# infil00p/openbts-ttsou

Measured on AMD Instinct MI355X. Metric: Mbursts/s (156.25-sym @ 4 sps) demod+detect, higher is better.
Workload: dtype f32

## Files before the change

openbts-ttsou_amd/csrc/trxsig_corr.h:

```cpp
#pragma once
#include "trxsig_dev.h"

namespace {

template <int SPS>
struct CorrGeom {
  static constexpr int NL = 36 * SPS;
  static constexpr int NC = (NL + 15) / 16;
  static constexpr int FRONT = 8 * SPS;
  static constexpr int WPAD0 = NC * 16 + 15 * SPS + 1;
  static constexpr int WPAD = ((WPAD0 + 15) / 32) * 32 + 16;
  static constexpr int H = (5 * SPS + 1 > 12) ? 5 * SPS + 1 : 12;
  static constexpr int NS = 2 * H + 1;
  static constexpr int NE = 20 * SPS;
  static constexpr int NEQ = (NE + 15) / 16;
  static constexpr int NPAIR = (NS + 2) / 2;
};
template <typename T>
__device__ __forceinline__ T &rec_slot(T *rec, int Bpad, int s, int b) { return rec[2 * ((size_t)(s >> 1) * Bpad + b) + (s & 1)]; }

template <int N>
__device__ __forceinline__ float add_row_shl(float acc, float v) {
  float r;
  if (N == 0) asm volatile("v_add_f32 %0, %1, %2" : "=v"(r) : "v"(v), "v"(acc));
  else asm volatile("v_add_f32_dpp %0, %1, %2 row_shl:%3 row_mask:0xf bank_mask:0xf bound_ctrl:1"
                    : "=v"(r) : "v"(v), "v"(acc), "n"(N));
  return r;
}
template <int SPS, int I>
__device__ __forceinline__ float energy_chain_step(float acc, const float (&nrm)[CorrGeom<SPS>::NEQ]) {
  if constexpr (I < CorrGeom<SPS>::NE) {
    acc = add_row_shl<I % 16>(acc, nrm[I / 16]);
    return energy_chain_step<SPS, I + 1>(acc, nrm);
  } else {
    return acc;
  }
}
template <int SPS, int I>
__device__ __forceinline__ float energy_chain(float acc, const float (&nrm)[CorrGeom<SPS>::NEQ]) {
  asm volatile("s_nop 1");
  return energy_chain_step<SPS, I>(acc, nrm);
}

template <int SPS>
struct CorrIn {
  typedef CorrGeom<SPS> G;
  static constexpr int NW = (CorrGeom<SPS>::NL + 15) / 16;
  cx w[NW];
  cx e[CorrGeom<SPS>::NEQ];
  int b;
  bool live, good;
  __device__ __forceinline__ void stage_window(cx *W, int r) const {
#pragma unroll
    for (int i = 0; i < NW; i++) {
      const int q = r + 16 * i;
      if (q < G::NL) W[G::FRONT + q] = w[i];
    }
  }
  __device__ __forceinline__ void stage_norms(float *ef, int r) const {
#pragma unroll
    for (int q = 0; q < G::NEQ; q++) {
      const int i = r + 16 * q;
      if (i < G::NE) ef[i] = norm2(e[q]);
    }
  }
};

template <int SPS>
__device__ __forceinline__ void corr_issue(CorrIn<SPS> &in, int b, int B, int r, const cx *__restrict__ samples,
                                           const int32_t *__restrict__ offset, const int32_t *__restrict__ length) {
  typedef CorrGeom<SPS> G;
  in.b = b;
  in.live = b < B;
  int off = 0, len = 0;
  if (in.live) { off = offset[b]; len = length[b]; }
  in.good = in.live && (off >= 0) && (len >= 92 * SPS) && (len <= 157 * SPS) && (len % SPS == 0);
  const cx *x = samples + (in.good ? off : 0);
#pragma unroll
  for (int i = 0; i < CorrIn<SPS>::NW; i++) {
    const int q = r + 16 * i;
    in.w[i] = (in.good && q < G::NL) ? x[56 * SPS + q] : mk(0, 0);
  }
#pragma unroll
  for (int q = 0; q < G::NEQ; q++) {
    const int i = r + 16 * q;
    in.e[q] = (in.good && i < G::NE) ? x[i] : mk(0, 0);
  }
}

template <int SPS, bool REC, bool EFIRST = false, unsigned TAPCLS = TRX_TAPS_GENERIC, typename IN = CorrIn<SPS>>
__device__ __forceinline__ void corr_round(const IN &in, cx *W, float4 *E, int lane, int r, const cx (&tap)[16],
                                           cx *__restrict__ rec, int Bpad, int &M_out, float &energy_out) {
  typedef CorrGeom<SPS> G;
  auto stage_norms = [&] { in.stage_norms(reinterpret_cast<float *>(E), r); };
  auto sum_norms = [&] {
    float energy = 0.0f;
#pragma unroll
    for (int i4 = 0; i4 < (G::NE + 3) / 4; i4++) {
      const float4 e = E[i4];
      energy = energy + e.x;
      if (4 * i4 + 1 < G::NE) energy = energy + e.y;
      if (4 * i4 + 2 < G::NE) energy = energy + e.z;
      if (4 * i4 + 3 < G::NE) energy = energy + e.w;
    }
    return energy;
  };
  float energy = 0.0f;
  if (EFIRST) {
    stage_norms();
    wave_lds_fence();
    energy = sum_norms();
    asm volatile("" : "+v"(energy));
    wave_lds_fence();
  }
  for (int q = r; q < G::FRONT; q += 16) W[q] = mk(0, 0);
  for (int q = G::FRONT + G::NL + r; q < G::WPAD; q += 16) W[q] = mk(0, 0);
  in.stage_window(W, r);
  if (!EFIRST) stage_norms();
  wave_lds_fence();
  if (!EFIRST) energy = sum_norms();

  float bestP = 0.0f;
  int bestT = -1;
  cx cval[G::NC];
  constexpr int CG = (SPS == 4) ? TRX_CORR_CG : 1;
  constexpr int UPC = 16 / SPS;
  constexpr int NU = UPC * (CG - 1) + 16;
#pragma unroll
  for (int c0 = 0; c0 < G::NC; c0 += CG) {
    cx sv[NU];
#pragma unroll
    for (int u = 0; u < NU; u++) sv[u] = W[r + 16 * c0 + SPS * u];
#pragma unroll
    for (int cc = 0; cc < CG; cc++) {
      if (c0 + cc < G::NC) {
        cx acc = mk(0, 0);
#pragma unroll
        for (int k = 15; k >= 0; k--) acc = cadd(acc, cmul_tap(sv[UPC * cc + k], tap[k], (TAPCLS >> (2 * k)) & 3));
        cval[c0 + cc] = acc;
      }
    }
  }
  wave_lds_fence();
#pragma unroll
  for (int c = 0; c < G::NC; c++) {
    const int t = r + 16 * c;
    if (t < G::NL) {
      W[t] = cval[c];
      const float p = norm2(cval[c]);
      if (p > bestP) { bestP = p; bestT = t; }
    }
  }
#pragma unroll
  for (int m = 1; m < 16; m <<= 1) {
    const float oP = __shfl_xor(bestP, m, 64);
    const int oT = __shfl_xor(bestT, m, 64);
    const bool take = (oP > bestP) || (oP == bestP && oT >= 0 && (bestT < 0 || oT < bestT));
    if (take) { bestP = oP; bestT = oT; }
  }
  wave_lds_fence();

  M_out = bestT;
  energy_out = energy;
  if (REC && in.live) {
    const int M = bestT;
    auto slot = [&](int s) {
      cx v = mk(0, 0);
      if (s < G::NS) {
        const int lag = M - G::H + s;
        if (lag >= 0 && lag < G::NL) v = W[lag];
      } else if (s == G::NS) {
        v = mk(__int_as_float(in.good ? M : -2), energy);
      }
      return v;
    };
    for (int j = r; j < G::NPAIR; j += 16) {
      const cx a = slot(2 * j), c = slot(2 * j + 1);
      reinterpret_cast<float4 *>(rec)[(size_t)j * Bpad + in.b] = make_float4(a.r, a.i, c.r, c.i);
    }
  }
  wave_lds_fence();
  (void)lane;
}


inline unsigned tap_classes(const TrxTables *hT, int tsc) {
  unsigned m = 0;
  for (int k = 0; k < 16; k++) {
    const trx_c32 a = hT->mid_ctap[tsc][k];
    const unsigned c = (a.r == 1.0f || a.r == -1.0f) ? 1u : ((a.i == 1.0f || a.i == -1.0f) ? 2u : 0u);
    m |= c << (2 * k);
  }
  return m;
}

}
```

openbts-ttsou_amd/csrc/trxsig_dev.h:

```cpp
#pragma once
#include <hip/hip_runtime.h>
#include <hip/hip_fp16.h>
#include <stdint.h>

#include <type_traits>

#include "trxsig_tables.h"
#include "trxsig_launch.h"

#ifndef TRX_CORR_CG
#define TRX_CORR_CG 3
#endif
#ifndef TRX_CORR_WPS
#define TRX_CORR_WPS 1
#endif
#ifndef TRX_CORR_ROUNDS
#define TRX_CORR_ROUNDS 1
#endif
#ifndef TRX_DEMOD_WAVES
#define TRX_DEMOD_WAVES 4
#endif

namespace {

typedef trx_c32 cx;

__device__ __forceinline__ cx mk(float r, float i) { cx z; z.r = r; z.i = i; return z; }
__device__ __forceinline__ cx cmul(cx x, cx a) { return mk(x.r * a.r - x.i * a.i, x.r * a.i + x.i * a.r); }
__device__ __forceinline__ cx cmulr(cx x, float a) { return mk(x.r * a, x.i * a); }
__device__ __forceinline__ cx cadd(cx x, cx a) { return mk(x.r + a.r, x.i + a.i); }
__device__ __forceinline__ float norm2(cx x) { return x.i * x.i + x.r * x.r; }
__device__ __forceinline__ cx cinv(cx x) { float n = norm2(x); return mk(x.r / n, -x.i / n); }
__device__ __forceinline__ cx cdiv(cx x, cx a) { return cmul(x, cinv(a)); }

template <int CTRL>
__device__ __forceinline__ float dpp_f(float v) {
  return __int_as_float(__builtin_amdgcn_update_dpp(0, __float_as_int(v), CTRL, 0xf, 0xf, true));
}
template <int CTRL>
__device__ __forceinline__ int dpp_i(int v) { return __builtin_amdgcn_update_dpp(0, v, CTRL, 0xf, 0xf, true); }
__device__ __forceinline__ float wave_sum_any_order(float v) {
  v += dpp_f<0xB1>(v);
  v += dpp_f<0x4E>(v);
  v += dpp_f<0x141>(v);
  v += dpp_f<0x140>(v);
  const float r0 = __int_as_float(__builtin_amdgcn_readlane(__float_as_int(v), 0));
  const float r1 = __int_as_float(__builtin_amdgcn_readlane(__float_as_int(v), 16));
  const float r2 = __int_as_float(__builtin_amdgcn_readlane(__float_as_int(v), 32));
  const float r3 = __int_as_float(__builtin_amdgcn_readlane(__float_as_int(v), 48));
  return ((r0 + r1) + r2) + r3;
}
__device__ __forceinline__ void argmax_take(float &P, int &T, float oP, int oT) {
  const bool take = (oP > P) || (oP == P && oT >= 0 && (T < 0 || oT < T));
  P = take ? oP : P;
  T = take ? oT : T;
}
__device__ __forceinline__ void wave_argmax(float &P, int &T) {
  argmax_take(P, T, dpp_f<0xB1>(P), dpp_i<0xB1>(T));
  argmax_take(P, T, dpp_f<0x4E>(P), dpp_i<0x4E>(T));
  argmax_take(P, T, dpp_f<0x141>(P), dpp_i<0x141>(T));
  argmax_take(P, T, dpp_f<0x140>(P), dpp_i<0x140>(T));
  float bp = __int_as_float(__builtin_amdgcn_readlane(__float_as_int(P), 0));
  int bt = __builtin_amdgcn_readlane(T, 0);
#pragma unroll
  for (int r = 16; r < 64; r += 16)
    argmax_take(bp, bt, __int_as_float(__builtin_amdgcn_readlane(__float_as_int(P), r)), __builtin_amdgcn_readlane(T, r));
  P = bp; T = bt;
}

typedef float v2f __attribute__((ext_vector_type(2)));
__device__ __forceinline__ v2f pk(cx z) { v2f v = {z.r, z.i}; return v; }
__device__ __forceinline__ v2f pk_cmul(v2f x, v2f a) {
  v2f p, q, r;
  asm("v_pk_mul_f32 %0, %1, %2 op_sel_hi:[0,1]" : "=v"(p) : "v"(x), "v"(a));
  asm("v_pk_mul_f32 %0, %1, %2 op_sel:[1,1] op_sel_hi:[1,0]" : "=v"(q) : "v"(x), "v"(a));
  asm("v_pk_add_f32 %0, %1, %2 neg_lo:[0,1]" : "=v"(r) : "v"(p), "v"(q));
  return r;
}
__device__ __forceinline__ v2f pk_mul(v2f x, v2f a) {
  v2f r;
  asm("v_pk_mul_f32 %0, %1, %2" : "=v"(r) : "v"(x), "v"(a));
  return r;
}
template <int HI>
__device__ __forceinline__ v2f pk_mul_tap(v2f x, v2f t) {
  v2f r;
  if (HI) asm("v_pk_mul_f32 %0, %1, %2 op_sel:[0,1] op_sel_hi:[1,1]" : "=v"(r) : "v"(x), "v"(t));
  else asm("v_pk_mul_f32 %0, %1, %2 op_sel_hi:[1,0]" : "=v"(r) : "v"(x), "v"(t));
  return r;
}
__device__ __forceinline__ v2f pk_csub(v2f x, v2f a) {
  v2f r;
  asm("v_pk_add_f32 %0, %1, %2 neg_lo:[0,1] neg_hi:[0,1]" : "=v"(r) : "v"(x), "v"(a));
  return r;
}
__device__ __forceinline__ cx unpk(v2f v) { return mk(v.x, v.y); }
__device__ __forceinline__ v2f pk_cadd(v2f x, v2f a) {
  v2f r;
  asm("v_pk_add_f32 %0, %1, %2" : "=v"(r) : "v"(x), "v"(a));
  return r;
}

struct SmpC32 {
  static constexpr int kBytes = 8;
  static __device__ __forceinline__ cx ld(const void *base, long long i) { return reinterpret_cast<const cx *>(base)[i]; }
  typedef cx raw_t;
  static __device__ __forceinline__ raw_t ldraw(const void *base, long long i) { return reinterpret_cast<const cx *>(base)[i]; }
  static __device__ __forceinline__ raw_t zero() { return mk(0, 0); }
  static __device__ __forceinline__ cx widen(raw_t r) { return r; }
  static __device__ __forceinline__ float4 ld2(const void *base, long long first, int q) {
    return reinterpret_cast<const float4 *>(reinterpret_cast<const cx *>(base) + first)[q];
  }
};
struct SmpF16 {
  static constexpr int kBytes = 4;
  static __device__ __forceinline__ cx ld(const void *base, long long i) {
    const float2 v = __half22float2(reinterpret_cast<const __half2 *>(base)[i]);
    return mk(v.x, v.y);
  }
  typedef unsigned raw_t;
  static __device__ __forceinline__ raw_t ldraw(const void *base, long long i) { return reinterpret_cast<const unsigned *>(base)[i]; }
  static __device__ __forceinline__ raw_t zero() { return 0u; }
  static __device__ __forceinline__ cx widen(raw_t r) {
    const float2 v = __half22float2(*reinterpret_cast<const __half2 *>(&r));
    return mk(v.x, v.y);
  }
  static __device__ __forceinline__ float4 ld2(const void *base, long long first, int q) {
    const uint2 u = reinterpret_cast<const uint2 *>(reinterpret_cast<const __half2 *>(base) + first)[q];
    const float2 a = __half22float2(*reinterpret_cast<const __half2 *>(&u.x)), b = __half22float2(*reinterpret_cast<const __half2 *>(&u.y));
    return make_float4(a.x, a.y, b.x, b.y);
  }
};

struct TapArg { float v[32]; };

#define TRX_TAPS_GENERIC 0u
template <int SPS> struct TapPattern {
  static constexpr unsigned value = (SPS == 4) ? 0x19999999u : 0x99999999u;
};
__device__ __forceinline__ float fma_steer(float a, float b, float c) {
  float r;
  asm("v_fma_f32 %0, %1, %2, %3 ; steering" : "=v"(r) : "v"(a), "v"(b), "v"(c));
  return r;
}
__device__ __forceinline__ float fma_steer_s(float a, float b_sgpr, float c) {
  float r;
  asm("v_fma_f32 %0, %1, %2, %3 ; steering" : "=v"(r) : "v"(a), "s"(b_sgpr), "v"(c));
  return r;
}
__device__ __forceinline__ cx cmul_tap(cx x, cx a, int cls) {
  if (cls == 1) {
    const float p = x.i * a.i, q = x.r * a.i;
    cx z;
    asm("v_fma_f32 %0, %2, %4, -%5 ; exact-product\n\tv_fma_f32 %1, %3, %4, %6 ; exact-product"
        : "=&v"(z.r), "=v"(z.i) : "v"(x.r), "v"(x.i), "s"(a.r), "v"(p), "v"(q));
    return z;
  }
  if (cls == 2) {
    const float p = x.r * a.r, q = x.i * a.r;
    cx z;
    asm("v_fma_f32 %0, %3, -%4, %5 ; exact-product\n\tv_fma_f32 %1, %2, %4, %6 ; exact-product"
        : "=&v"(z.r), "=v"(z.i) : "v"(x.r), "v"(x.i), "s"(a.i), "v"(p), "v"(q));
    return z;
  }
  return cmul(x, a);
}

#define TRX_PI_F 3.14159274101257324f
#define TRX_2PI_F 6.28318548202514648f

template <int N>
__device__ __forceinline__ float row_shl(float v) {
  if (N == 0) return v;
  return __int_as_float(__builtin_amdgcn_update_dpp(0, __float_as_int(v), 0x100 + N, 0xf, 0xf, true));
}

__device__ __forceinline__ void lds_barrier() {
  asm volatile("s_waitcnt lgkmcnt(0)\n\ts_barrier" ::: "memory");
}
__device__ __forceinline__ void wave_lds_fence() {
  __builtin_amdgcn_fence(__ATOMIC_RELEASE, "wavefront");
  __builtin_amdgcn_wave_barrier();
  __builtin_amdgcn_fence(__ATOMIC_ACQUIRE, "wavefront");
}

__device__ __forceinline__ float dev_range_reduce(float arg) {
  if (arg > 1.0F) arg = arg - (ceilf(arg) - 1.0F);
  if (arg < 0.0F) arg = arg + ceilf(-arg);
  return arg;
}
__device__ __forceinline__ float dev_sin_lookup(const float *__restrict__ sinT, float x) {
  const float arg = dev_range_reduce(x * (1 / TRX_2PI_F));
  const float argT = arg * (float)TRX_TABLESIZE;
  int argI = (int)argT;
  argI = argI < 0 ? 0 : (argI > TRX_TABLESIZE ? TRX_TABLESIZE : argI);
  const float delta = argT - argI;
  const float iDelta = 1.0F - delta;
  return iDelta * sinT[argI] + delta * sinT[argI + 1];
}
#define TRX_FSHIFT_MAXPHASE 25000.0f
__device__ __forceinline__ cx dev_expj_lookup(const TrxTables *__restrict__ T, float x) {
  const float arg = dev_range_reduce(x * (1 / TRX_2PI_F));
  const float argT = arg * (float)TRX_TABLESIZE;
  int argI = (int)argT;
  argI = argI < 0 ? 0 : (argI > TRX_TABLESIZE ? TRX_TABLESIZE : argI);
  const float delta = argT - argI;
  const float iDelta = 1.0F - delta;
  return mk(iDelta * T->cosT[argI] + delta * T->cosT[argI + 1], iDelta * T->sinT[argI] + delta * T->sinT[argI + 1]);
}
__device__ __forceinline__ float dev_sinc(const float *__restrict__ sinT, float x) {
  if ((x >= 0.01F) || (x <= -0.01F)) return dev_sin_lookup(sinT, x) / x;
  return 1.0F;
}

}
```

openbts-ttsou_amd/csrc/trxsig_normal.hip:

```cpp
#include "trxsig_bisect.h"
#include "trxsig_corr.h"
#include "trxsig_demod.h"
#include "trxsig_rxgen.h"

#ifndef TRX_RXC_WPS
#define TRX_RXC_WPS 1
#endif
#ifndef TRX_RXD_WPS
#define TRX_RXD_WPS 1
#endif

namespace {

template <int SPS, unsigned TAPCLS>
__global__ __launch_bounds__(256, TRX_CORR_WPS) void k_tsc_corr(const TrxTables *__restrict__ T,
                                                  const cx *__restrict__ samples,
                                                  const int32_t *__restrict__ offset,
                                                  const int32_t *__restrict__ length, int B, TapArg taps,
                                                  cx *__restrict__ rec, int Bpad) {
  typedef CorrGeom<SPS> G;
  static_assert(8 * G::WPAD >= 4 * G::NE, "the energy norms are staged in the row itself");
  __shared__ __attribute__((aligned(16))) cx rows[16][G::WPAD];
  (void)T;
  const int lane = threadIdx.x & 63, wave = threadIdx.x >> 6;
  const int row = lane >> 4, r = lane & 15;
  const int slot = wave * 4 + row;

  cx tap[16];
#pragma unroll
  for (int k = 0; k < 16; k++) tap[k] = mk(taps.v[2 * k], taps.v[2 * k + 1]);

  typedef CorrIn<SPS> In;
  In in[TRX_CORR_ROUNDS];
#pragma unroll
  for (int i = 0; i < TRX_CORR_ROUNDS; i++)
    corr_issue<SPS>(in[i], (blockIdx.x * TRX_CORR_ROUNDS + i) * 16 + slot, B, r, samples, offset, length);
#pragma unroll
  for (int i = 0; i < TRX_CORR_ROUNDS; i++) {
    int M;
    float energy;
    corr_round<SPS, true, true, TAPCLS, In>(in[i], rows[slot], reinterpret_cast<float4 *>(rows[slot]), lane, r, tap, rec, Bpad, M, energy);
  }
}


#ifdef TRX_TUNING_BUILD
template <int SPS>
__global__ __launch_bounds__(64) void k_tsc_peak(const TrxTables *__restrict__ T,
                                                 const cx *__restrict__ rec, int Bpad, int B, int tsc,
                                                 float detect_thresh, float energy_thresh,
                                                 uint8_t *__restrict__ flags, cx *__restrict__ amp_out,
                                                 float *__restrict__ toa_out,
                                                 float *__restrict__ avgpwr_out) {
  typedef CorrGeom<SPS> G;
  __shared__ cx loc[26][64];
  __shared__ float pw[G::NS][64];
  const int lane = threadIdx.x;
  const int b = blockIdx.x * 64 + lane;
  const bool live = b < B;
  const int bb = live ? b : B - 1;

  const cx meta = rec_slot(rec, Bpad, G::NS, bb);
  const int M = __float_as_int(meta.r);
  const float energy = meta.i;
  const bool good = M != -2;
#pragma unroll
  for (int s = 0; s < G::NS; s++) {
    const cx v = rec_slot(rec, Bpad, s, bb);
    pw[s][lane] = norm2(v);
    const int j = s - (G::H - 12);
    if (j >= 0 && j < 24) {
      const int lag = M - 12 + j;
      loc[j][lane] = (lag > G::NL - 2) ? mk(0, 0) : v;
    }
  }
  loc[24][lane] = mk(0, 0);
  loc[25][lane] = mk(0, 0);

  float peakIx;
  const cx peak = peak_bisect<64>(T->sinc_grid, loc, lane, M, &peakIx);

  float toa = peakIx;
  cx amp = peak;
  bool detected = false;
  const bool energy_ok = good && (energy_thresh < 0.0f ||
                                  energy / (float)(unsigned)G::NE > energy_thresh * energy_thresh);
  if (!(toa < 0.0f) && !(toa > (float)G::NL) && good) {
    const int p = (int)rintf(toa);
    float valley = 0.0f;
    int numRms = 0;
#pragma unroll
    for (int i = 2 * SPS; i <= 5 * SPS; i++) {
      const int lo = p - i, hi = p + i;
      int slo = lo - M + G::H, shi = hi - M + G::H;
      slo = slo < 0 ? 0 : slo; shi = shi > G::NS - 1 ? G::NS - 1 : shi;
      const float vlo = pw[slo][lane], vhi = pw[shi][lane];
      if (lo >= 0) { valley += vlo; numRms++; }
      if (hi < G::NL) { valley += vhi; numRms++; }
    }
    if (numRms < 2) {
      amp = mk(0, 0);
    } else {
      const float RMS = (float)((double)sqrtf(valley / (float)numRms) + 0.00001);
      const float peakToMean = sqrtf(norm2(amp)) / RMS;
      amp = cdiv(amp, T->mid_gain[tsc]);
      toa = toa - T->mid_toa[tsc];
      toa = toa - (float)((66 - 56) * SPS);
      detected = peakToMean > detect_thresh;
    }
  } else {
    amp = mk(0, 0);
  }
  if (!energy_ok) { amp = mk(0, 0); toa = 0.0f; detected = false; }

  if (live) {
    uint8_t fl = 0;
    if (!good) fl = TRXSIG_F_BADLEN;
    else fl = (energy_ok ? TRXSIG_F_ENERGY : 0) | (detected ? TRXSIG_F_DETECT : 0);
    flags[b] = fl;
    amp_out[b] = amp;
    toa_out[b] = toa;
    if (avgpwr_out) avgpwr_out[b] = good ? energy / (float)(unsigned)G::NE : 0.0f;
  }
}


template <int SPS>
struct Peak8Geom {
  typedef CorrGeom<SPS> G;
  static constexpr int NV = 2 * (3 * SPS + 1);
  static constexpr int O_PW = 26 * 2;
  static constexpr int O_V = O_PW + ((G::NS + 3) & ~3);
  static constexpr int STRIDE = O_V + ((NV + 3) & ~3);
};

template <int SPS>
__global__ __launch_bounds__(256, 8) void k_tsc_peak8(const TrxTables *__restrict__ T, const cx *__restrict__ rec, int Bpad,
                                                   int B, cx gain_inv, float mid_toa, float detect_thresh,
                                                   float energy_thresh, uint8_t *__restrict__ flags,
                                                   cx *__restrict__ amp_out, float *__restrict__ toa_out,
                                                   float *__restrict__ avgpwr_out) {
  typedef CorrGeom<SPS> G;
  typedef Peak8Geom<SPS> P8;
  __shared__ __attribute__((aligned(16))) float stab[32][24];
  __shared__ __attribute__((aligned(16))) float scratch[32][P8::STRIDE];
  {
    float tv[3];
#pragma unroll
    for (int k = 0; k < 3; k++) { const int ix = threadIdx.x * 3 + k; tv[k] = T->sinc_grid[16 * (ix / 24)][ix % 24]; }
#pragma unroll
    for (int k = 0; k < 3; k++) { const int ix = threadIdx.x * 3 + k; stab[ix / 24][ix % 24] = tv[k]; }
  }
  const int lane = threadIdx.x & 63;
  const int r = lane & 7;
  const int slot = threadIdx.x >> 3;
  const int b = blockIdx.x * 32 + slot;
  const bool live = b < B;
  const int bb = live ? b : B - 1;
  float *S = scratch[slot];
  cx *loc = reinterpret_cast<cx *>(S);
  float *pw = S + P8::O_PW, *V = S + P8::O_V;

  const cx meta = rec_slot(rec, Bpad, G::NS, bb);
  const int M = __float_as_int(meta.r);
  const float energy = meta.i;
  const bool good = M != -2;
#pragma unroll
  for (int s0 = 0; s0 < G::NS; s0 += 8) {
    const int sl = s0 + r;
    if (sl < G::NS) {
      const cx v = rec_slot(rec, Bpad, sl, bb);
      pw[sl] = norm2(v);
      const int j = sl - (G::H - 12);
      if (j >= 0 && j < 24) loc[j] = (M - 12 + j > G::NL - 2) ? mk(0, 0) : v;
    }
  }
  if (r < 2) loc[24 + r] = mk(0, 0);
  __syncthreads();

  int e = 0;
  asm volatile("" : "+v"(e));
  bool active = true;
  cx peak = mk(0, 0);
  {
    const int rel2 = kFusedRel2.v[r], rel1 = kFusedRel1.v[r];
#pragma unroll
    for (int st = 0; st < 4; st++) {
      const int inc_last = 128 >> (2 * st);
      const int el = e + (rel2 >> 2) * inc_last;
      float srow[24];
      if (st < 3) {
        const float4 *rw = reinterpret_cast<const float4 *>(stab[(el & 511) >> 4]);
#pragma unroll
        for (int q = 0; q < 6; q++) {
          const float4 t4 = rw[q];
          srow[4 * q] = t4.x; srow[4 * q + 1] = t4.y; srow[4 * q + 2] = t4.z; srow[4 * q + 3] = t4.w;
        }
      } else {
        fused_row(T, el, srow);
      }
      const cx pt = fused_point(loc, el, rel2 & 3, srow);
      fused_decide<8, 2, false>(pt, lane, 2 * inc_last, e, active, peak);
    }
    {
      float srow[24];
      fused_row(T, e, srow);
      const cx pt = fused_point(loc, e, rel1 & 3, srow);
      fused_decide<8, 1, false>(pt, lane, 1, e, active, peak);
    }
    float srow[24];
    fused_row(T, e, srow);
    peak = fused_point(loc, e, 1, srow);
    asm volatile("" : "+v"(peak.r), "+v"(peak.i));
  }
  cx amp;
  float toa;
  bool detected, energy_ok;
  fused_tail<SPS, 8>([&](int lag) { const int sl = lag - M + G::H; return (sl < 0 || sl >= G::NS) ? 0.0f : pw[sl]; }, V, r, M, e,
                     peak, good, energy, gain_inv, mid_toa, detect_thresh, energy_thresh, amp, toa, detected, energy_ok);
  if (live && r == 0) {
    uint8_t fl = 0;
    if (!good) fl = TRXSIG_F_BADLEN;
    else fl = (energy_ok ? TRXSIG_F_ENERGY : 0) | (detected ? TRXSIG_F_DETECT : 0);
    flags[b] = fl;
    amp_out[b] = amp;
    toa_out[b] = toa;
    if (avgpwr_out) avgpwr_out[b] = good ? energy / (float)(unsigned)G::NE : 0.0f;
  }
}



#endif

#ifndef TRX_PEAK2_THREADS
#define TRX_PEAK2_THREADS 512
#endif
constexpr int kPeak2Threads = TRX_PEAK2_THREADS;
template <int SPS>
__global__ __launch_bounds__(kPeak2Threads) void k_tsc_peak2(const TrxTables *__restrict__ T, const cx *__restrict__ rec, int Bpad,
                                                   int B, cx gain_inv, float mid_toa, float detect_thresh,
                                                   float energy_thresh, uint8_t *__restrict__ flags,
                                                   cx *__restrict__ amp_out, float *__restrict__ toa_out,
                                                   float *__restrict__ avgpwr_out) {
  typedef CorrGeom<SPS> G;
  constexpr int NL = G::NL, NE = G::NE, NP = 3 * SPS + 3;
  __shared__ __attribute__((aligned(16))) SincLds stab;
  const int tid = threadIdx.x;
  const int h = tid & 1;
  const int b = blockIdx.x * (kPeak2Threads / 2) + (tid >> 1);
  const bool live = b < B;
  const int bb = live ? b : B - 1;
#ifdef TRX_PEAK_PROBE
  long long pt_[16] = {0};
  int pk_ = 0;
#define TRX_STAMP() pt_[pk_++] = clock64()
#else
#define TRX_STAMP()
#endif
  TRX_STAMP();

  float4 tv[3072 / kPeak2Threads];
  sinc_lds_issue<kPeak2Threads>(T, tid, tv);
  const cx meta = rec_slot(rec, Bpad, G::NS, bb);
  const int M = __float_as_int(meta.r);
  const float energy = meta.i;
  const bool good = M != -2;
  const float4 *rec4 = reinterpret_cast<const float4 *>(rec);
  cx q[23];
  {
    constexpr int S0 = G::H - 12, P0 = S0 >> 1;
    float4 pw[12];
#pragma unroll
    for (int i = 0; i < 12; i++) pw[i] = rec4[(size_t)(P0 + h + i) * Bpad + bb];
#pragma unroll
    for (int k = 0; k < 23; k++) {
      const int ix = k + 2 * h;
      const float4 p4 = pw[((S0 + k) >> 1) - P0];
      const cx v = ((S0 + k) & 1) ? mk(p4.z, p4.w) : mk(p4.x, p4.y);
      q[k] = (M - 12 + ix > NL - 2) ? mk(0, 0) : v;
    }
  }
  cx vmine_[NP];
  constexpr int VLO = G::H - (5 * SPS + 1), VHI = G::H + (2 * SPS - 1);
  if constexpr ((VLO & 1) == 0 && (VHI & 1) == 0) {
    float4 pv[(NP + 1) / 2];
#pragma unroll
    for (int i = 0; i < (NP + 1) / 2; i++) pv[i] = rec4[(size_t)(((h ? VHI : VLO) >> 1) + i) * Bpad + bb];
#pragma unroll
    for (int k = 0; k < NP; k++) vmine_[k] = (k & 1) ? mk(pv[k >> 1].z, pv[k >> 1].w) : mk(pv[k >> 1].x, pv[k >> 1].y);
  } else {
#pragma unroll
    for (int k = 0; k < NP; k++) vmine_[k] = rec_slot(rec, Bpad, (h ? VHI : VLO) + k, bb);
  }
  sinc_lds_store<kPeak2Threads>(stab, tid, tv);
  TRX_STAMP();
  __syncthreads();
  TRX_STAMP();

  int e;
  const cx peak = pair_bisect(stab, q, h, e);
  TRX_STAMP();
  const float early = (float)(M - 1) + (float)e * 0.001953125f;
  float toa = early + 1.0f;
  cx amp = peak;
  bool detected = false;
  const bool energy_ok = good && (energy_thresh < 0.0f || energy / (float)(unsigned)NE > energy_thresh * energy_thresh);
  const bool sane = !(toa < 0.0f) && !(toa > (float)NL) && good;
  if (sane) {
    const int pk = (int)rintf(toa);
    const int a = pk - M + 1;
    float plo[NP], phi[NP];
#pragma unroll
    for (int k = 0; k < NP; k++) {
      const float mine = norm2(vmine_[k]);
      const float other = __int_as_float(__builtin_amdgcn_update_dpp(0, __float_as_int(mine), 0xB1, 0xf, 0xf, true));
      plo[k] = h ? other : mine; phi[k] = h ? mine : other;
    }
    float valley = 0.0f;
#pragma unroll
    for (int i = 2 * SPS; i <= 5 * SPS; i++) {
      const int t = 5 * SPS - i, u = i - 2 * SPS;
      const float vlo = a == 0 ? plo[t] : (a == 1 ? plo[t + 1] : plo[t + 2]);
      const float vhi = a == 0 ? phi[u] : (a == 1 ? phi[u + 1] : phi[u + 2]);
      valley = valley + vlo;
      valley = valley + vhi;
    }
    int nlo = (pk < 5 * SPS ? pk : 5 * SPS) - 2 * SPS + 1;
    int nhi = (NL - 1 - pk < 5 * SPS ? NL - 1 - pk : 5 * SPS) - 2 * SPS + 1;
    nlo = nlo < 0 ? 0 : nlo; nhi = nhi < 0 ? 0 : nhi;
    const int numRms = nlo + nhi;
    if (numRms < 2) {
      amp = mk(0, 0);
    } else {
      const float RMS = (float)((double)sqrtf(valley / (float)numRms) + 0.00001);
      const float peakToMean = sqrtf(norm2(amp)) / RMS;
      amp = cmul(amp, gain_inv);
      toa = toa - mid_toa;
      toa = toa - (float)((66 - 56) * SPS);
      detected = peakToMean > detect_thresh;
    }
  } else {
    amp = mk(0, 0);
  }
  if (!energy_ok) { amp = mk(0, 0); toa = 0.0f; detected = false; }

  if (live && h == 0) {
    uint8_t fl = 0;
    if (!good) fl = TRXSIG_F_BADLEN;
    else fl = (energy_ok ? TRXSIG_F_ENERGY : 0) | (detected ? TRXSIG_F_DETECT : 0);
    flags[b] = fl;
    amp_out[b] = amp;
    toa_out[b] = toa;
    if (avgpwr_out) avgpwr_out[b] = good ? energy / (float)(unsigned)G::NE : 0.0f;
  }
#ifdef TRX_PEAK_PROBE
  TRX_STAMP();
  if (live && avgpwr_out) {
    long long v = 0;
    for (int k = 1; k < 16; k++) if ((b & 15) == k) v = pt_[k] - pt_[0];
    if (h == 0) avgpwr_out[b] = (float)v;
  }
#endif
#undef TRX_STAMP
}

template <int SPS, unsigned TAPCLS>
__global__ __launch_bounds__(256, TRX_RXC_WPS) void k_tsc_corr_rx(TrxRxGen a, int B, TapArg taps, cx *__restrict__ rec, int Bpad) {
  static_assert(SPS == 4, "the fused front end is the 260 : 96 resampler");
  typedef CorrGeom<SPS> G;
  constexpr int XCAP = 160;
  static_assert(G::WPAD >= XCAP, "the raw stretch is parked in the burst's own row");
  __shared__ __attribute__((aligned(16))) cx rows[16][G::WPAD];
  __shared__ float4 tpb_s[RXG_NT];
  if (threadIdx.x < RXG_NT) tpb_s[threadIdx.x] = a.tpb[threadIdx.x];
  __syncthreads();
  const int lane = threadIdx.x & 63, wave = threadIdx.x >> 6;
  const int row = lane >> 4, r = lane & 15;
  const int slot = wave * 4 + row;
  cx tap[16];
#pragma unroll
  for (int k = 0; k < 16; k++) tap[k] = mk(taps.v[2 * k], taps.v[2 * k + 1]);
  const int b = blockIdx.x * 16 + slot;
  CorrIn<SPS> in;
  in.b = b; in.live = b < B; in.good = in.live;
  const RxBurst u = rx_burst(a, in.live ? b : 0);
  const int jlo = rx_index(u.g0, a.skipD).j0 - 3;
  cx *X = rows[slot];
  {
    short2 v[XCAP / 16];
#pragma unroll
    for (int i = 0; i < XCAP / 16; i++) v[i] = rx_raw(a, u.s, jlo + r + 16 * i);
#pragma unroll
    for (int i = 0; i < XCAP / 16; i++) X[r + 16 * i] = rx_widen(a, v[i]);
  }
  wave_lds_fence();
  {
    static_assert(G::NL % 16 == 0 && G::NE % 16 == 0, "every lane owns a sample in every round");
    const int nb = rx_boundary(u.g0);
    RxIdx ix = rx_index(u.g0 + 56 * SPS + r, a.skipD);
#pragma unroll
    for (int i = 0; i < CorrIn<SPS>::NW; i++) {
      in.w[i] = rx_sample(X, tpb_s, jlo, ix, nb - (56 * SPS + r + 16 * i), a.w0, a.w1);
      ix = rx_step<16>(ix);
      if (i % 3 == 2) asm volatile("" : "+v"(in.w[i].r), "+v"(in.w[i].i), "+v"(in.w[i - 1].r), "+v"(in.w[i - 1].i), "+v"(in.w[i - 2].r), "+v"(in.w[i - 2].i) : : "memory");
    }
    ix = rx_index(u.g0 + r, a.skipD);
#pragma unroll
    for (int q = 0; q < G::NEQ; q++) {
      in.e[q] = rx_sample(X, tpb_s, jlo, ix, nb - (r + 16 * q), a.w0, a.w1);
      ix = rx_step<16>(ix);
      if (q % 3 == 2) asm volatile("" : "+v"(in.e[q].r), "+v"(in.e[q].i), "+v"(in.e[q - 1].r), "+v"(in.e[q - 1].i), "+v"(in.e[q - 2].r), "+v"(in.e[q - 2].i) : : "memory");
    }
  }
  wave_lds_fence();
  int M;
  float energy;
  corr_round<SPS, true, true, TAPCLS>(in, rows[slot], reinterpret_cast<float4 *>(rows[slot]), lane, r, tap, rec, Bpad, M, energy);
}

template <int SPS, bool TOL = false>
__global__ __launch_bounds__(64 * TRX_DEMOD_WAVES, TRX_RXD_WPS) void k_demod_rx(const TrxTables *__restrict__ T, TrxRxGen a, int B,
                                                                  const cx *__restrict__ amp_in, const float *__restrict__ toa_in,
                                                                  const uint8_t *__restrict__ flags, int need_mask,
                                                                  float *__restrict__ soft, uint8_t *__restrict__ hard, int nsoft,
                                                                  int stride) {
  static_assert(SPS == 4, "the fused front end is the 260 : 96 resampler");
  typedef DemodGeom<SPS, 148> G;
  constexpr int XCAP = 256;
  static_assert(G::U >= XCAP, "the raw stretch is parked in the burst's staging area");
  __shared__ cx ph[TRX_DEMOD_WAVES][G::U];
  __shared__ float4 tpb_s[RXG_NT];
  if (threadIdx.x < RXG_NT) tpb_s[threadIdx.x] = a.tpb[threadIdx.x];
  __syncthreads();
  const int lane = threadIdx.x & 63;
  const int wave = __builtin_amdgcn_readfirstlane(threadIdx.x >> 6);
  const int b = blockIdx.x * TRX_DEMOD_WAVES + wave;
  if (b >= B) return;
  float *sb = soft + (size_t)b * stride;
  uint8_t *hb = hard ? hard + (size_t)b * stride : nullptr;
  const cx amp = amp_in[b];
  const float toa = toa_in[b];
  bool enabled = fabsf(toa) <= 4096.0f;
  if (flags) enabled = enabled && (need_mask ? ((flags[b] & need_mask) == need_mask) : (flags[b] != 0));
  if (!enabled) {
    for (int m = lane; m < nsoft; m += 64) { sb[m] = 0.0f; if (hb) hb[m] = 0; }
    return;
  }
  const RxBurst u = rx_burst(a, b);
  const int jlo = rx_index(u.g0, a.skipD).j0 - 3;
  cx *X = ph[wave];
  {
    short2 v[XCAP / 64];
#pragma unroll
    for (int i = 0; i < XCAP / 64; i++) v[i] = rx_raw(a, u.s, jlo + lane + 64 * i);
#pragma unroll
    for (int i = 0; i < XCAP / 64; i++) X[lane + 64 * i] = rx_widen(a, v[i]);
  }
  wave_lds_fence();
  constexpr int NSL = (157 * SPS + 63) / 64;
  cx sv[NSL];
  {
    const int nb = rx_boundary(u.g0);
    RxIdx ix = rx_index(u.g0 + lane, a.skipD);
#pragma unroll
    for (int i = 0; i < NSL; i++) {
      sv[i] = rx_sample(X, tpb_s, jlo, ix, nb - (lane + 64 * i), a.w0, a.w1);
      ix = rx_step<64>(ix);
      if (i % 2 == 1) asm volatile("" : "+v"(sv[i].r), "+v"(sv[i].i), "+v"(sv[i - 1].r), "+v"(sv[i - 1].i) : : "memory");
    }
  }
  const int N = u.N;
  auto stage = [&](cx *P, cx inv, int lo) {
    typedef DemodGeom<SPS, 148> D;
    const int u0 = lane + lo;
    if (u0 >= 0) {
      cx *p0 = P + (u0 % SPS) * D::QLEN + u0 / SPS;
#pragma unroll
      for (int i = 0; i < NSL; i++)
        if (lane + 64 * i < N && u0 + 64 * i < D::U) p0[i * (64 / SPS)] = cmul(sv[i], inv);
    } else {
#pragma unroll
      for (int i = 0; i < NSL; i++) {
        const int uu = u0 + 64 * i;
        if (lane + 64 * i < N && uu >= 0 && uu < D::U) P[(uu % SPS) * D::QLEN + uu / SPS] = cmul(sv[i], inv);
      }
    }
  };
  if (TOL) {
    float xm = 0.0f;
#pragma unroll
    for (int i = 0; i < NSL; i++)
      if (lane + 64 * i < N) xm = max3_abs(sv[i].r, sv[i].i, xm);
    auto stage_raw = [&](cx *P, int lo) {
      typedef DemodGeom<SPS, 148> D;
      const int u0 = lane + lo;
      if (u0 >= 0) {
        cx *p0 = P + (u0 % SPS) * D::QLEN + u0 / SPS;
#pragma unroll
        for (int i = 0; i < NSL; i++)
          if (lane + 64 * i < N && u0 + 64 * i < D::U) p0[i * (64 / SPS)] = sv[i];
      } else {
#pragma unroll
        for (int i = 0; i < NSL; i++) {
          const int uu = u0 + 64 * i;
          if (lane + 64 * i < N && uu >= 0 && uu < D::U) P[(uu % SPS) * D::QLEN + uu / SPS] = sv[i];
        }
      }
    };
    if (fused_demod_tol_ex<SPS>(T, ph[wave], N, amp, toa, lane, sb, hb, nsoft, xm, stage_raw)) return;
  }
  fused_demod_ex<SPS, 64>(T, ph[wave], N, amp, toa, lane, sb, hb, nsoft, stage, [] {}, nullptr, nullptr);
}

}

int trx_rec_slots(int sps) {
  switch (sps) {
    case 1: return 2 * CorrGeom<1>::NPAIR;
    case 2: return 2 * CorrGeom<2>::NPAIR;
    case 4: return 2 * CorrGeom<4>::NPAIR;
  }
  return 0;
}

template <int S>
static void launch_tsc_detect(hipStream_t st, const TrxTables *dT, const TrxTables *hT, const trx_c32 *samples, const int32_t *off,
                              const int32_t *len, int B, int tsc, float detect_thresh, float energy_thresh,
                              trx_c32 *rec, int Bpad, uint8_t *flags, trx_c32 *amp, float *toa, float *avgpwr,
                              int variant, TrxProfiler *prof) {
  TapArg ta;
  for (int k = 0; k < 16; k++) { ta.v[2 * k] = hT->mid_ctap[tsc][k].r; ta.v[2 * k + 1] = hT->mid_ctap[tsc][k].i; }
  if (prof) prof->begin(TRXSIG_K_TSC_CORR, st);
  const dim3 cgrid((B + 16 * TRX_CORR_ROUNDS - 1) / (16 * TRX_CORR_ROUNDS));
  if (!(variant & 1) && tap_classes(hT, tsc) == TapPattern<S>::value)
    k_tsc_corr<S, TapPattern<S>::value><<<cgrid, dim3(256), 0, st>>>(dT, samples, off, len, B, ta, rec, Bpad);
  else
    k_tsc_corr<S, TRX_TAPS_GENERIC><<<cgrid, dim3(256), 0, st>>>(dT, samples, off, len, B, ta, rec, Bpad);
  if (prof) { prof->end(TRXSIG_K_TSC_CORR, st); prof->begin(TRXSIG_K_TSC_PEAK, st); }
  const trx_c32 g = hT->mid_gain[tsc];
  const float n = g.i * g.i + g.r * g.r;
  trx_c32 ginv; ginv.r = g.r / n; ginv.i = -g.i / n;
#ifdef TRX_TUNING_BUILD
  if (variant & 4) {
    k_tsc_peak<S><<<dim3((B + 63) / 64), dim3(64), 0, st>>>(dT, rec, Bpad, B, tsc, detect_thresh, energy_thresh,
                                                            flags, amp, toa, avgpwr);
  } else if (variant & 2) {
    k_tsc_peak8<S><<<dim3((B + 31) / 32), dim3(256), 0, st>>>(dT, rec, Bpad, B, ginv, hT->mid_toa[tsc], detect_thresh,
                                                              energy_thresh, flags, amp, toa, avgpwr);
  } else
#endif
  {
    k_tsc_peak2<S><<<dim3((B + kPeak2Threads / 2 - 1) / (kPeak2Threads / 2)), dim3(kPeak2Threads), 0, st>>>(dT, rec, Bpad, B, ginv, hT->mid_toa[tsc], detect_thresh,
                                                                energy_thresh, flags, amp, toa, avgpwr);
  }
  if (prof) prof->end(TRXSIG_K_TSC_PEAK, st);
}

namespace {
__global__ __launch_bounds__(256) void k_copy_verdict(const uint8_t *__restrict__ f, const cx *__restrict__ a, const float *__restrict__ t, int B,
                                                      uint8_t *__restrict__ fo, cx *__restrict__ ao, float *__restrict__ to) {
  const int b = blockIdx.x * 256 + threadIdx.x;
  if (b >= B) return;
  fo[b] = f[b]; ao[b] = a[b]; to[b] = t[b];
}
}
hipError_t trx_launch_copy_verdict(hipStream_t st, const uint8_t *flags, const trx_c32 *amp, const float *toa, int B, uint8_t *flags_out,
                                   trx_c32 *amp_out, float *toa_out) {
  if (B <= 0) return hipSuccess;
  k_copy_verdict<<<dim3((B + 255) / 256), dim3(256), 0, st>>>(flags, amp, toa, B, flags_out, amp_out, toa_out);
  return hipGetLastError();
}

hipError_t trx_launch_tsc_detect(hipStream_t st, int sps, const TrxTables *dT, const TrxTables *hT, const trx_c32 *samples,
                                 const int32_t *off, const int32_t *len, int B, int tsc,
                                 float detect_thresh, float energy_thresh, trx_c32 *rec, int Bpad,
                                 uint8_t *flags, trx_c32 *amp, float *toa, float *avgpwr, int variant,
                                 TrxProfiler *prof) {
  if (B <= 0) return hipSuccess;
  switch (sps) {
    case 1: launch_tsc_detect<1>(st, dT, hT, samples, off, len, B, tsc, detect_thresh, energy_thresh, rec, Bpad, flags, amp, toa, avgpwr, variant, prof); break;
    case 2: launch_tsc_detect<2>(st, dT, hT, samples, off, len, B, tsc, detect_thresh, energy_thresh, rec, Bpad, flags, amp, toa, avgpwr, variant, prof); break;
    case 4: launch_tsc_detect<4>(st, dT, hT, samples, off, len, B, tsc, detect_thresh, energy_thresh, rec, Bpad, flags, amp, toa, avgpwr, variant, prof); break;
    default: return hipErrorInvalidValue;
  }
  return hipGetLastError();
}

hipError_t trx_launch_rx_normal(hipStream_t st, const TrxTables *dT, const TrxTables *hT, const TrxRxGen &gen, int B, int tsc,
                                float detect_thresh, float energy_thresh, trx_c32 *rec, int Bpad, uint8_t *flags, trx_c32 *amp,
                                float *toa, float *avgpwr, float *soft, uint8_t *hard, int nsoft, int stride, int generic_taps,
                                TrxProfiler *prof, int soft_tolerance) {
  if (B <= 0) return hipSuccess;
  if (nsoft > 148 || gen.nb <= 0) return hipErrorInvalidValue;
  constexpr int S = 4;
  TapArg ta;
  for (int k = 0; k < 16; k++) { ta.v[2 * k] = hT->mid_ctap[tsc][k].r; ta.v[2 * k + 1] = hT->mid_ctap[tsc][k].i; }
  if (prof) prof->begin(TRXSIG_K_TSC_CORR, st);
  const dim3 cgrid((B + 15) / 16);
  if (!generic_taps && tap_classes(hT, tsc) == TapPattern<S>::value)
    k_tsc_corr_rx<S, TapPattern<S>::value><<<cgrid, dim3(256), 0, st>>>(gen, B, ta, rec, Bpad);
  else
    k_tsc_corr_rx<S, TRX_TAPS_GENERIC><<<cgrid, dim3(256), 0, st>>>(gen, B, ta, rec, Bpad);
  if (prof) { prof->end(TRXSIG_K_TSC_CORR, st); prof->begin(TRXSIG_K_TSC_PEAK, st); }
  const trx_c32 g = hT->mid_gain[tsc];
  const float n = g.i * g.i + g.r * g.r;
  trx_c32 ginv; ginv.r = g.r / n; ginv.i = -g.i / n;
  k_tsc_peak2<S><<<dim3((B + kPeak2Threads / 2 - 1) / (kPeak2Threads / 2)), dim3(kPeak2Threads), 0, st>>>(dT, rec, Bpad, B, ginv, hT->mid_toa[tsc], detect_thresh, energy_thresh,
                                                              flags, amp, toa, avgpwr);
  if (prof) prof->end(TRXSIG_K_TSC_PEAK, st);
  if (nsoft > 0) {
    if (prof) prof->begin(TRXSIG_K_DEMOD, st);
    if (soft_tolerance)
      k_demod_rx<S, true><<<dim3((B + TRX_DEMOD_WAVES - 1) / TRX_DEMOD_WAVES), dim3(64 * TRX_DEMOD_WAVES), 0, st>>>(
          dT, gen, B, amp, toa, flags, TRXSIG_F_DETECT, soft, hard, nsoft, stride);
    else
      k_demod_rx<S><<<dim3((B + TRX_DEMOD_WAVES - 1) / TRX_DEMOD_WAVES), dim3(64 * TRX_DEMOD_WAVES), 0, st>>>(
          dT, gen, B, amp, toa, flags, TRXSIG_F_DETECT, soft, hard, nsoft, stride);
    if (prof) prof->end(TRXSIG_K_DEMOD, st);
  }
  return hipGetLastError();
}

hipError_t trx_launch_rx_demod(hipStream_t st, const TrxTables *dT, const TrxRxGen &gen, int B, const trx_c32 *amp, const float *toa,
                               const uint8_t *flags, int need_mask, float *soft, uint8_t *hard, int nsoft, int stride, TrxProfiler *prof,
                               int soft_tolerance) {
  if (B <= 0 || nsoft <= 0) return hipSuccess;
  if (nsoft > 148 || gen.nb <= 0) return hipErrorInvalidValue;
  if (prof) prof->begin(TRXSIG_K_DEMOD, st);
  if (soft_tolerance)
    k_demod_rx<4, true><<<dim3((B + TRX_DEMOD_WAVES - 1) / TRX_DEMOD_WAVES), dim3(64 * TRX_DEMOD_WAVES), 0, st>>>(dT, gen, B, amp, toa, flags,
                                                                                                                  need_mask, soft, hard, nsoft, stride);
  else
    k_demod_rx<4><<<dim3((B + TRX_DEMOD_WAVES - 1) / TRX_DEMOD_WAVES), dim3(64 * TRX_DEMOD_WAVES), 0, st>>>(dT, gen, B, amp, toa, flags, need_mask,
                                                                                                            soft, hard, nsoft, stride);
  if (prof) prof->end(TRXSIG_K_DEMOD, st);
  return hipGetLastError();
}

hipError_t trx_launch_demod(hipStream_t st, int sps, const TrxTables *dT, const trx_c32 *samples,
                            const int32_t *off, const int32_t *len, int B, const trx_c32 *amp,
                            const float *toa, const uint8_t *flags, int need_mask, float *soft,
                            uint8_t *hard, int nsoft, int stride, TrxProfiler *prof, int soft_tolerance) {
  if (B <= 0) return hipSuccess;
  const dim3 grid((B + TRX_DEMOD_WAVES - 1) / TRX_DEMOD_WAVES), block(64 * TRX_DEMOD_WAVES);
  if (prof) prof->begin(TRXSIG_K_DEMOD, st);
#define TRX_DEMOD_CASE(S)                                                                                          \
  case S:                                                                                                          \
    if (nsoft <= 148 && soft_tolerance)                                                                            \
      k_demod<S, false, 148, SmpC32, true><<<grid, block, 0, st>>>(dT, samples, off, len, B, amp, toa, flags, need_mask, soft, hard, \
                                                     nsoft, stride);                                              \
    else if (nsoft <= 148)                                                                                         \
      k_demod<S, false, 148><<<grid, block, 0, st>>>(dT, samples, off, len, B, amp, toa, flags, need_mask, soft, hard, \
                                                     nsoft, stride);                                              \
    else                                                                                                           \
      k_demod<S, false, 157><<<grid, block, 0, st>>>(dT, samples, off, len, B, amp, toa, flags, need_mask, soft, hard, \
                                                     nsoft, stride);                                              \
    break;
  switch (sps) {
    TRX_DEMOD_CASE(1)
    TRX_DEMOD_CASE(2)
    TRX_DEMOD_CASE(4)
    default: return hipErrorInvalidValue;
  }
#undef TRX_DEMOD_CASE
  if (prof) prof->end(TRXSIG_K_DEMOD, st);
  return hipGetLastError();
}
```

Measured before the change: 635.8.

## Pack correlator LDS rows contiguously, gate energy sums, raise occupancy bounds

Replaces the per-burst padded LDS rows with one contiguous buffer whose row stride is chosen so adjacent rows sit 32 dwords apart, shrinking LDS per block and zeroing only the gaps between windows. Adds an energy mode that skips staging and summing exact sample norms when avgpwr is not requested and a cheap wave-reduced sum already decides the threshold test, substituting infinity or the partial value. Raises launch-bounds waves-per-SIMD for the correlation kernels so more blocks can be resident. The gating depends on carefully derived rounding constants, and the higher occupancy bounds may force register spills.

```diff
diff --git a/openbts-ttsou_amd/csrc/trxsig_corr.h b/openbts-ttsou_amd/csrc/trxsig_corr.h
--- a/openbts-ttsou_amd/csrc/trxsig_corr.h
+++ b/openbts-ttsou_amd/csrc/trxsig_corr.h
@@ -10,6 +10,11 @@
   static constexpr int FRONT = 8 * SPS;
   static constexpr int WPAD0 = NC * 16 + 15 * SPS + 1;
   static constexpr int WPAD = ((WPAD0 + 15) / 32) * 32 + 16;
+  static constexpr int GAP0 = (WPAD0 - FRONT - NL > FRONT) ? WPAD0 - FRONT - NL : FRONT;
+  static constexpr int GAP = GAP0 + ((16 - (NL + GAP0)) % 32 + 32) % 32;
+  static constexpr int RSTRIDE = NL + GAP;
+  static constexpr int ROWS_LEN = 16 * RSTRIDE + GAP;
+  static_assert(RSTRIDE % 32 == 16 && GAP % 2 == 0 && RSTRIDE % 2 == 0, "rows 32 dwords apart (mod 64), windows 16-byte aligned");
   static constexpr int H = (5 * SPS + 1 > 12) ? 5 * SPS + 1 : 12;
   static constexpr int NS = 2 * H + 1;
   static constexpr int NE = 20 * SPS;
@@ -88,10 +93,22 @@
   }
 }
 
+constexpr int TRX_E_EXACT = 0, TRX_E_GATE = 1, TRX_E_OFF = 2;
+inline int corr_energy_mode(const float *avgpwr, float energy_thresh) {
+  if (avgpwr) return TRX_E_EXACT;
+  if (energy_thresh >= 0.0f) return TRX_E_GATE;
+  return energy_thresh < 0.0f ? TRX_E_OFF : TRX_E_EXACT;
+}
+
+constexpr float TRX_EGATE_KHI = 0x1.9998p-7f, TRX_EGATE_KLO = 0x1.999b34p-7f;
+constexpr float TRX_EGATE_SMIN = 0x1p-100f, TRX_EGATE_SMAX = 0x1p126f;
+
 template <int SPS, bool REC, bool EFIRST = false, unsigned TAPCLS = TRX_TAPS_GENERIC, typename IN = CorrIn<SPS>>
 __device__ __forceinline__ void corr_round(const IN &in, cx *W, float4 *E, int lane, int r, const cx (&tap)[16],
-                                           cx *__restrict__ rec, int Bpad, int &M_out, float &energy_out) {
+                                           cx *__restrict__ rec, int Bpad, int &M_out, float &energy_out,
+                                           int emode = TRX_E_EXACT, float ethr = 0.0f) {
   typedef CorrGeom<SPS> G;
+  constexpr int CO = REC ? G::FRONT : 0;
   auto stage_norms = [&] { in.stage_norms(reinterpret_cast<float *>(E), r); };
   auto sum_norms = [&] {
     float energy = 0.0f;
@@ -107,14 +124,45 @@
   };
   float energy = 0.0f;
   if (EFIRST) {
-    stage_norms();
-    wave_lds_fence();
-    energy = sum_norms();
-    asm volatile("" : "+v"(energy));
-    wave_lds_fence();
-  }
-  for (int q = r; q < G::FRONT; q += 16) W[q] = mk(0, 0);
-  for (int q = G::FRONT + G::NL + r; q < G::WPAD; q += 16) W[q] = mk(0, 0);
+    bool need = emode == TRX_E_EXACT;
+    float stand_in = 0.0f;
+    if (emode == TRX_E_GATE) {
+      float s = norm2(in.e[0]);
+#pragma unroll
+      for (int q = 1; q < G::NEQ; q++) s = s + (r + 16 * q < G::NE ? norm2(in.e[q]) : 0.0f);
+      s = s + dpp_f<0xB1>(s);
+      s = s + dpp_f<0x4E>(s);
+      s = s + dpp_f<0x141>(s);
+      s = s + dpp_f<0x140>(s);
+      const float T = ethr * ethr;
+      constexpr float KHI = TRX_EGATE_KHI * (float)(80 / G::NE), KLO = TRX_EGATE_KLO * (float)(80 / G::NE);
+      static_assert(80 % G::NE == 0 && G::NE - 1 <= 79 && G::NEQ <= 5, "the gate's constants are derived for these");
+      need = true;
+      if (s == 0.0f) {
+        need = false;
+      } else if (s >= TRX_EGATE_SMIN && s <= TRX_EGATE_SMAX) {
+        if (s * KHI > T) { need = false; stand_in = __builtin_inff(); }
+        else if (s * KLO <= T) need = false;
+      }
+    }
+    if (emode == TRX_E_EXACT || (emode == TRX_E_GATE && __any(need))) {
+      stage_norms();
+      wave_lds_fence();
+      energy = sum_norms();
+      asm volatile("" : "+v"(energy));
+      wave_lds_fence();
+    }
+    energy = need ? energy : stand_in;
+  }
+  if (REC) {
+    for (int q = r; q < G::GAP; q += 16) {
+      W[G::FRONT - G::GAP + q] = mk(0, 0);
+      W[G::FRONT + G::NL + q] = mk(0, 0);
+    }
+  } else {
+    for (int q = r; q < G::FRONT; q += 16) W[q] = mk(0, 0);
+    for (int q = G::FRONT + G::NL + r; q < G::WPAD; q += 16) W[q] = mk(0, 0);
+  }
   in.stage_window(W, r);
   if (!EFIRST) stage_norms();
   wave_lds_fence();
@@ -146,7 +194,7 @@
   for (int c = 0; c < G::NC; c++) {
     const int t = r + 16 * c;
     if (t < G::NL) {
-      W[t] = cval[c];
+      W[CO + t] = cval[c];
       const float p = norm2(cval[c]);
       if (p > bestP) { bestP = p; bestT = t; }
     }
@@ -168,7 +216,7 @@
       cx v = mk(0, 0);
       if (s < G::NS) {
         const int lag = M - G::H + s;
-        if (lag >= 0 && lag < G::NL) v = W[lag];
+        if (lag >= 0 && lag < G::NL) v = W[CO + lag];
       } else if (s == G::NS) {
         v = mk(__int_as_float(in.good ? M : -2), energy);
       }
diff --git a/openbts-ttsou_amd/csrc/trxsig_dev.h b/openbts-ttsou_amd/csrc/trxsig_dev.h
--- a/openbts-ttsou_amd/csrc/trxsig_dev.h
+++ b/openbts-ttsou_amd/csrc/trxsig_dev.h
@@ -12,7 +12,7 @@
 #define TRX_CORR_CG 3
 #endif
 #ifndef TRX_CORR_WPS
-#define TRX_CORR_WPS 1
+#define TRX_CORR_WPS 7
 #endif
 #ifndef TRX_CORR_ROUNDS
 #define TRX_CORR_ROUNDS 1
diff --git a/openbts-ttsou_amd/csrc/trxsig_normal.hip b/openbts-ttsou_amd/csrc/trxsig_normal.hip
--- a/openbts-ttsou_amd/csrc/trxsig_normal.hip
+++ b/openbts-ttsou_amd/csrc/trxsig_normal.hip
@@ -4,7 +4,7 @@
 #include "trxsig_rxgen.h"
 
 #ifndef TRX_RXC_WPS
-#define TRX_RXC_WPS 1
+#define TRX_RXC_WPS 6
 #endif
 #ifndef TRX_RXD_WPS
 #define TRX_RXD_WPS 1
@@ -13,18 +13,19 @@
 namespace {
 
 template <int SPS, unsigned TAPCLS>
-__global__ __launch_bounds__(256, TRX_CORR_WPS) void k_tsc_corr(const TrxTables *__restrict__ T,
+__global__ __launch_bounds__(256, TAPCLS == TRX_TAPS_GENERIC ? 6 : TRX_CORR_WPS) void k_tsc_corr(const TrxTables *__restrict__ T,
                                                   const cx *__restrict__ samples,
                                                   const int32_t *__restrict__ offset,
                                                   const int32_t *__restrict__ length, int B, TapArg taps,
-                                                  cx *__restrict__ rec, int Bpad) {
+                                                  cx *__restrict__ rec, int Bpad, int emode, float ethr) {
   typedef CorrGeom<SPS> G;
-  static_assert(8 * G::WPAD >= 4 * G::NE, "the energy norms are staged in the row itself");
-  __shared__ __attribute__((aligned(16))) cx rows[16][G::WPAD];
+  static_assert(2 * G::NL >= G::NE, "the energy norms are staged in the row itself");
+  __shared__ __attribute__((aligned(16))) cx rows[G::ROWS_LEN];
   (void)T;
   const int lane = threadIdx.x & 63, wave = threadIdx.x >> 6;
   const int row = lane >> 4, r = lane & 15;
   const int slot = wave * 4 + row;
+  cx *W = rows + G::GAP - G::FRONT + slot * G::RSTRIDE;
 
   cx tap[16];
 #pragma unroll
@@ -39,7 +40,8 @@
   for (int i = 0; i < TRX_CORR_ROUNDS; i++) {
     int M;
     float energy;
-    corr_round<SPS, true, true, TAPCLS, In>(in[i], rows[slot], reinterpret_cast<float4 *>(rows[slot]), lane, r, tap, rec, Bpad, M, energy);
+    corr_round<SPS, true, true, TAPCLS, In>(in[i], W, reinterpret_cast<float4 *>(W + G::FRONT), lane, r, tap, rec, Bpad, M, energy,
+                                            emode, ethr);
   }
 }
 
@@ -366,12 +368,14 @@
 }
 
 template <int SPS, unsigned TAPCLS>
-__global__ __launch_bounds__(256, TRX_RXC_WPS) void k_tsc_corr_rx(TrxRxGen a, int B, TapArg taps, cx *__restrict__ rec, int Bpad) {
+__global__ __launch_bounds__(256, TRX_RXC_WPS) void k_tsc_corr_rx(TrxRxGen a, int B, TapArg taps, cx *__restrict__ rec, int Bpad,
+                                                                   int emode, float ethr) {
   static_assert(SPS == 4, "the fused front end is the 260 : 96 resampler");
   typedef CorrGeom<SPS> G;
   constexpr int XCAP = 160;
-  static_assert(G::WPAD >= XCAP, "the raw stretch is parked in the burst's own row");
-  __shared__ __attribute__((aligned(16))) cx rows[16][G::WPAD];
+  constexpr int XSTR = 168;
+  static_assert(3 * XSTR + XCAP <= 3 * G::RSTRIDE + G::NL, "the raw stretches stay inside the wave's own rows");
+  __shared__ __attribute__((aligned(16))) cx rows[G::ROWS_LEN];
   __shared__ float4 tpb_s[RXG_NT];
   if (threadIdx.x < RXG_NT) tpb_s[threadIdx.x] = a.tpb[threadIdx.x];
   __syncthreads();
@@ -386,7 +390,8 @@
   in.b = b; in.live = b < B; in.good = in.live;
   const RxBurst u = rx_burst(a, in.live ? b : 0);
   const int jlo = rx_index(u.g0, a.skipD).j0 - 3;
-  cx *X = rows[slot];
+  cx *W = rows + G::GAP - G::FRONT + slot * G::RSTRIDE;
+  cx *X = rows + G::GAP + 4 * wave * G::RSTRIDE + row * XSTR;
   {
     short2 v[XCAP / 16];
 #pragma unroll
@@ -416,7 +421,7 @@
   wave_lds_fence();
   int M;
   float energy;
-  corr_round<SPS, true, true, TAPCLS>(in, rows[slot], reinterpret_cast<float4 *>(rows[slot]), lane, r, tap, rec, Bpad, M, energy);
+  corr_round<SPS, true, true, TAPCLS>(in, W, reinterpret_cast<float4 *>(W + G::FRONT), lane, r, tap, rec, Bpad, M, energy, emode, ethr);
 }
 
 template <int SPS, bool TOL = false>
@@ -533,10 +538,11 @@
   for (int k = 0; k < 16; k++) { ta.v[2 * k] = hT->mid_ctap[tsc][k].r; ta.v[2 * k + 1] = hT->mid_ctap[tsc][k].i; }
   if (prof) prof->begin(TRXSIG_K_TSC_CORR, st);
   const dim3 cgrid((B + 16 * TRX_CORR_ROUNDS - 1) / (16 * TRX_CORR_ROUNDS));
+  const int emode = corr_energy_mode(avgpwr, energy_thresh);
   if (!(variant & 1) && tap_classes(hT, tsc) == TapPattern<S>::value)
-    k_tsc_corr<S, TapPattern<S>::value><<<cgrid, dim3(256), 0, st>>>(dT, samples, off, len, B, ta, rec, Bpad);
+    k_tsc_corr<S, TapPattern<S>::value><<<cgrid, dim3(256), 0, st>>>(dT, samples, off, len, B, ta, rec, Bpad, emode, energy_thresh);
   else
-    k_tsc_corr<S, TRX_TAPS_GENERIC><<<cgrid, dim3(256), 0, st>>>(dT, samples, off, len, B, ta, rec, Bpad);
+    k_tsc_corr<S, TRX_TAPS_GENERIC><<<cgrid, dim3(256), 0, st>>>(dT, samples, off, len, B, ta, rec, Bpad, emode, energy_thresh);
   if (prof) { prof->end(TRXSIG_K_TSC_CORR, st); prof->begin(TRXSIG_K_TSC_PEAK, st); }
   const trx_c32 g = hT->mid_gain[tsc];
   const float n = g.i * g.i + g.r * g.r;
@@ -598,10 +604,11 @@
   for (int k = 0; k < 16; k++) { ta.v[2 * k] = hT->mid_ctap[tsc][k].r; ta.v[2 * k + 1] = hT->mid_ctap[tsc][k].i; }
   if (prof) prof->begin(TRXSIG_K_TSC_CORR, st);
   const dim3 cgrid((B + 15) / 16);
+  const int emode = corr_energy_mode(avgpwr, energy_thresh);
   if (!generic_taps && tap_classes(hT, tsc) == TapPattern<S>::value)
-    k_tsc_corr_rx<S, TapPattern<S>::value><<<cgrid, dim3(256), 0, st>>>(gen, B, ta, rec, Bpad);
+    k_tsc_corr_rx<S, TapPattern<S>::value><<<cgrid, dim3(256), 0, st>>>(gen, B, ta, rec, Bpad, emode, energy_thresh);
   else
-    k_tsc_corr_rx<S, TRX_TAPS_GENERIC><<<cgrid, dim3(256), 0, st>>>(gen, B, ta, rec, Bpad);
+    k_tsc_corr_rx<S, TRX_TAPS_GENERIC><<<cgrid, dim3(256), 0, st>>>(gen, B, ta, rec, Bpad, emode, energy_thresh);
   if (prof) { prof->end(TRXSIG_K_TSC_CORR, st); prof->begin(TRXSIG_K_TSC_PEAK, st); }
   const trx_c32 g = hT->mid_gain[tsc];
   const float n = g.i * g.i + g.r * g.r;
```

New measurement: 641.8 (median of 6 runs). No clear change (+0.9%).
